# stnamjef/GenerativeDensification

Hardware: AMD Instinct MI355X
Metric: views/sec fwd+bwd @ 800x800 (higher is better)
Workload: dtype f32; 1 GPU; c4: BASELINE configs[3] per-GPU share: 2M densified-like Gaussians, 4 views/GPU 800x800, SH3, fwd+bwd; n_gaussians=2000000, layout=cube, order=random, views_per_gpu=4, sh_degree=3, parallelism=view-sharded x1, grad_allreduce=False, entry=render_views (all views of the shard, one node), activations fused into K1/K9, loss=folded into K6 epilogue / K7 prologue (clamp+MSE+0.1 mean depth+0.1 mean alpha)

## Files before the change

### generativedensification_amd/_debug.py

```python
import os as _os


def _int_env(name):
    return int(_os.environ[name]) if _os.environ.get(name) else None


RENDER_SIDE = int(_os.environ.get("GDR_RENDER_SIDE", "1"))
FWD_STREAMS = int(_os.environ.get("GDR_FWD_STREAMS", "4"))
BWD_STREAMS = _int_env("GDR_BWD_STREAMS")
BIN_STREAM = None
K7_VIEWS = _int_env("GDR_K7_VIEWS")
EARLY_CLEAR = True

SEG_LEN = _int_env("GDR_SEG_LEN")
DEEP_MAX_BUSY = None
DEEP_MIN_MEAN = _int_env("GDR_DEEP_MIN_MEAN")
FORCE_GLOBAL_SORT = False
SCATTER_MODE = int(_os.environ.get("GDR_SCATTER_MODE", "0"))
FORCE_RADIX_PARTITION = False
LAUNCH_HINTS = True

DEFER_D = _os.environ.get("GDR_DEFER_D", "1") != "0"
```

### generativedensification_amd/_lib.py

```python
from __future__ import annotations

import ctypes as C
import os

import torch

_HERE = os.path.dirname(os.path.abspath(__file__))
LIB_PATH = os.environ.get("GDR_LIB_PATH") or os.path.join(_HERE, "lib", "libgdr_hip.so")

GDR_OK = 0
GDR_IN_RAW_OPACITY, GDR_IN_RAW_SCALES, GDR_IN_RAW_ROTATIONS, GDR_IN_NO_DEPTH_TO_MEAN = 1, 2, 4, 8
GDR_MAX_VIEWS = 8
GDR_MAX_NODE_VIEWS = 256
ABI_VERSION = 17
GDR_SAME_AS_MAX, GDR_REUSE_MAX = 8, 32
GDR_DEFAULT_SEG_LEN = 256
GDR_ERR_WORKSPACE = -4


class GdrSettings(C.Structure):
    _fields_ = [("image_height", C.c_int32), ("image_width", C.c_int32), ("tanfovx", C.c_float),
                ("tanfovy", C.c_float), ("scale_modifier", C.c_float), ("sh_degree", C.c_int32),
                ("prefiltered", C.c_int32), ("debug", C.c_int32), ("bg", C.c_void_p),
                ("viewmatrix", C.c_void_p), ("projmatrix", C.c_void_p), ("campos", C.c_void_p)]
# ... 136 lines not shown
    _fields_ = [("N", C.c_int64), ("V", C.c_int32), ("C", C.c_int32), ("H", C.c_int32), ("W", C.c_int32),
                ("reserved", C.c_int32)]


GDR_SUBM_DTYPES = {"f16": 0, "bf16": 1, "f32": 2}
GDR_SUBM_MAX_TAPS, GDR_SUBM_MAX_CHANNELS, GDR_SUBM_MAX_POINTS = 125, 512, 1 << 30


GDR_SEG_ROWS, GDR_SEG_MAX_CHANNELS = 32, 65536
GDR_SEG_DTYPES = {"f16": 0, "bf16": 1, "f32": 2, "i64": 3}
GDR_SEG_OPS = {"sum": 0, "mean": 1, "min": 2, "max": 3}

GDR_NORM_DTYPES = {"f16": 0, "bf16": 1, "f32": 2}
GDR_NORM_ROWS, GDR_NORM_MAX_CHANNELS, GDR_NORM_MAX_SEGMENTS, GDR_NORM_MAX_FREQS, GDR_NORM_MAX_UPSCALE = 32, 1024, 1024, 16, 16


class GdrSubmArgs(C.Structure):
    _fields_ = [("N", C.c_int32), ("Cin", C.c_int32), ("Cout", C.c_int32), ("K", C.c_int32), ("dtype", C.c_int32),
                ("reserved", C.c_int32)]


_PROTOS = {
    "gdr_abi_version": (C.c_int, []),
    "gdr_last_error": (C.c_char_p, []),
    "gdr_geom_bytes": (C.c_size_t, [C.c_int32]),
    "gdr_binning_bytes": (C.c_size_t, [C.c_uint64]),
    "gdr_image_bytes": (C.c_size_t, [C.c_int32, C.c_int32]),
    "gdr_geom_carve": (C.c_int, [C.c_void_p, C.c_int32, C.POINTER(GdrGeom)]),
    "gdr_binning_carve": (C.c_int, [C.c_void_p, C.c_uint64, C.POINTER(GdrBinning)]),
    "gdr_binning_bytes_for": (C.c_size_t, [C.c_uint64, C.c_int32, C.c_int32, C.c_int32]),
    "gdr_binning_carve_for": (C.c_int, [C.c_void_p, C.c_uint64, C.c_int32, C.c_int32, C.c_int32, C.POINTER(GdrBinning)]),
    "gdr_build_tag": (C.c_char_p, []),
    "gdr_set_scatter_mode": (C.c_int32, [C.c_int32]),
    "gdr_words_differ": (C.c_int, [C.c_void_p, C.c_void_p, C.c_uint64, C.c_void_p, C.c_void_p]),
    "gdr_words_differ_multi": (C.c_int, [C.c_int32, C.POINTER(C.c_void_p), C.POINTER(C.c_void_p), C.POINTER(C.c_uint64), C.c_void_p,
                                         C.c_void_p]),
    "gdr_host_copy_begin": (C.c_int, [C.c_void_p, C.c_void_p, C.c_uint64, C.c_void_p, C.POINTER(C.c_void_p)]),
    "gdr_host_copy_wait": (C.c_int, [C.c_void_p]),
    "gdr_clear_async": (C.c_int, [C.c_void_p, C.c_uint64, C.c_void_p]),
    "gdr_image_carve": (C.c_int, [C.c_void_p, C.c_int32, C.c_int32, C.POINTER(GdrImage)]),
    "gdr_preprocess_forward": (C.c_int, [C.POINTER(GdrSettings), C.POINTER(GdrInputs), C.POINTER(GdrGeom),
                                         C.c_void_p, C.POINTER(C.c_uint32), C.c_void_p]),
    "gdr_render_forward": (C.c_int, [C.POINTER(GdrSettings), C.POINTER(GdrInputs), C.POINTER(GdrGeom),
                                     C.POINTER(GdrBinning), C.POINTER(GdrImage), C.c_uint64,
                                     C.POINTER(GdrOutputs), C.c_void_p]),
    "gdr_binning_forward": (C.c_int, [C.POINTER(GdrSettings), C.c_int32, C.POINTER(GdrGeom), C.POINTER(GdrBinning),
                                      C.POINTER(GdrImage), C.c_uint64, C.c_void_p, C.c_void_p]),
    "gdr_composite_forward": (C.c_int, [C.POINTER(GdrSettings), C.POINTER(GdrGeom), C.POINTER(GdrBinning),
                                        C.POINTER(GdrImage), C.POINTER(GdrOutputs), C.c_void_p]),
    "gdr_composite_forward_loss": (C.c_int, [C.POINTER(GdrSettings), C.POINTER(GdrGeom), C.POINTER(GdrBinning),
                                             C.POINTER(GdrImage), C.POINTER(GdrOutputs), C.c_void_p, C.c_float, C.c_float,
                                             C.c_void_p, C.c_void_p]),
    "gdr_composite_forward_views": (C.c_int, [C.c_int32, C.POINTER(GdrSettings), C.POINTER(GdrGeom), C.POINTER(GdrBinning),
                                              C.POINTER(GdrImage), C.POINTER(GdrOutputs), C.c_int32, C.POINTER(C.c_void_p),
                                              C.c_float, C.c_float, C.c_float, C.c_void_p, C.c_int32, C.c_void_p]),
    "gdr_render_backward_loss": (C.c_int, [C.POINTER(GdrSettings), C.c_int32, C.POINTER(GdrGeom), C.POINTER(GdrBinning),
                                           C.POINTER(GdrImage), C.c_void_p, C.c_void_p, C.c_float, C.c_float, C.c_void_p,
                                           C.c_void_p, C.c_void_p]),
    "gdr_forward": (C.c_int, [C.POINTER(GdrSettings), C.POINTER(GdrInputs), C.POINTER(GdrGeom),
                              C.POINTER(GdrBinning), C.POINTER(GdrImage), C.c_uint64,
                              C.POINTER(GdrOutputs), C.POINTER(C.c_uint32), C.c_void_p]),
    "gdr_view_plan_for": (C.c_int, [C.c_int32, C.c_int32, C.c_int32, C.c_int32, C.c_uint64, C.POINTER(GdrViewOpts),
                                    C.POINTER(GdrViewPlan)]),
    "gdr_forward_view": (C.c_int, [C.POINTER(GdrSettings), C.POINTER(GdrInputs), C.POINTER(GdrViewPlan), C.c_void_p,
                                   C.POINTER(GdrViewOpts), C.POINTER(GdrSameAs), C.POINTER(GdrOutputs),
                                   C.POINTER(GdrViewState), C.c_void_p]),
# ... 240 lines not shown
```

### generativedensification_amd/csrc/api.hip

```cpp
#include <stdio.h>
#include <string.h>

#include <atomic>
#include <cmath>
#include <mutex>
#include <unordered_map>
#include <vector>

#include "gdr_common.h"
#include "host_util.h"

namespace gdr {

static thread_local char g_err[512] = "";

void set_error(const char* what, hipError_t e) {
    snprintf(g_err, sizeof(g_err), "%s: %s (%d)", what, e == hipSuccess ? "" : hipGetErrorString(e), (int)e);
}

struct ProfRec { int id; hipEvent_t a, b; };
static bool g_prof_on = false;
static std::vector<ProfRec> g_prof_pending;
static std::vector<hipEvent_t> g_prof_pool;
static double g_prof_ms[GDR_K_COUNT];
// ... 264 lines not shown
        if (in->shs) {
            if (s->sh_degree < 0 || s->sh_degree > 3) { set_error("sh_degree must be 0..3", hipSuccess); return GDR_ERR_UNSUPPORTED; }
            if (in->M < (s->sh_degree + 1) * (s->sh_degree + 1)) { set_error("M < (sh_degree+1)^2", hipSuccess); return GDR_ERR_INVALID_ARG; }
            if (!s->campos) { set_error("campos NULL", hipSuccess); return GDR_ERR_INVALID_ARG; }
        }
    }
    return GDR_OK;
}

static int hip_fail(const char* what, hipError_t e) {
    set_error(what, e);
    return GDR_ERR_HIP;
}

static int debug_sync(const gdr_settings* s, const char* what, hipStream_t st) {
    if (!s->debug) return GDR_OK;
    hipError_t e = hipStreamSynchronize(st);
    if (e != hipSuccess) return hip_fail(what, e);
    return GDR_OK;
}

}

using namespace gdr;

extern "C" {

int gdr_abi_version(void) { return GDR_ABI_VERSION; }
#ifndef GDR_BUILD_TAG
#define GDR_BUILD_TAG "release"
#endif
const char* gdr_build_tag(void) { return GDR_BUILD_TAG; }
int32_t gdr_set_scatter_mode(int32_t mode) { return set_scatter_mode_default(mode); }
const char* gdr_last_error(void) { return g_err; }

size_t gdr_geom_bytes(int32_t N) { return carve_geom(nullptr, N, nullptr); }
size_t gdr_binning_bytes(uint64_t D) { return carve_binning(nullptr, D, nullptr); }
size_t gdr_image_bytes(int32_t H, int32_t W) { return carve_image(nullptr, H, W, nullptr); }

int gdr_geom_carve(void* base, int32_t N, gdr_geom* out) {
    if (!base || !out || ((uintptr_t)base & 255u)) { set_error("geom base NULL/unaligned", hipSuccess); return GDR_ERR_INVALID_ARG; }
    carve_geom(base, N, out);
    return GDR_OK;
}
int gdr_binning_carve(void* base, uint64_t D, gdr_binning* out) {
    if (!base || !out || ((uintptr_t)base & 255u)) { set_error("binning base NULL/unaligned", hipSuccess); return GDR_ERR_INVALID_ARG; }
    carve_binning(base, D, out);
    return GDR_OK;
}
size_t gdr_binning_bytes_for(uint64_t D, int32_t seg_len, int32_t N, int32_t tiles) {
    return carve_binning(nullptr, D, nullptr, seg_len, N, tiles);
}
int gdr_binning_carve_for(void* base, uint64_t D, int32_t seg_len, int32_t N, int32_t tiles, gdr_binning* out) {
    if (!base || !out || ((uintptr_t)base & 255u) || seg_len < 0 || N < 0 || tiles < 0) {
        set_error("binning base NULL/unaligned or negative seg_len / N / tiles", hipSuccess);
        return GDR_ERR_INVALID_ARG;
    }
    carve_binning(base, D, out, seg_len, N, tiles);
    return GDR_OK;
}
int gdr_image_carve(void* base, int32_t H, int32_t W, gdr_image* out) {
    if (!base || !out || ((uintptr_t)base & 255u)) { set_error("image base NULL/unaligned", hipSuccess); return GDR_ERR_INVALID_ARG; }
    carve_image(base, H, W, out);
    return GDR_OK;
}

// ... 1501 lines not shown
```

### generativedensification_amd/csrc/binning.hip

```cpp
#include <string.h>
#include <atomic>

#include "gdr_common.h"

namespace gdr {

namespace {

__device__ __forceinline__ uint32_t lane_id() { return threadIdx.x & 63u; }
__device__ __forceinline__ uint64_t lanemask_lt() { return (1ull << lane_id()) - 1ull; }

__device__ __forceinline__ uint32_t wave_incl_scan(uint32_t v) {
#pragma unroll
    for (int off = 1; off < 64; off <<= 1) {
        uint32_t t = __shfl_up(v, off, 64);
        if ((int)lane_id() >= off) v += t;
    }
    return v;
}

__device__ __forceinline__ uint32_t block_excl_scan(uint32_t v, uint32_t* lds, uint32_t* total) {
    const uint32_t incl = wave_incl_scan(v);
    const uint32_t w = threadIdx.x >> 6;
    if (lane_id() == 63) lds[w] = incl;
// ... 598 lines not shown
            uint32_t j = i + 1;
            while (j < L && kA[j] == kA[i]) ++j;
            if (j - i > GDR_TIE_SERIAL) {
                const uint32_t slot = atomicAdd(&runs[2 * GDR_TIE_RUNS], 1u);
                if (slot < GDR_TIE_RUNS) { runs[2 * slot] = i; runs[2 * slot + 1] = j - i; continue; }
            }
            for (uint32_t a = i + 1; a < j; ++a) {
                const uint32_t x = vA[a];
                uint32_t c = a;
                while (c > i && vA[c - 1] > x) { vA[c] = vA[c - 1]; --c; }
                vA[c] = x;
            }
        }
    }
    __syncthreads();
    const uint32_t nruns = min(runs[2 * GDR_TIE_RUNS], (uint32_t)GDR_TIE_RUNS);
    for (uint32_t r = 0; r < nruns; ++r) {
        const uint32_t i0 = runs[2 * r], Lr = runs[2 * r + 1];
        if constexpr (EPT > 0) {
            for (int shift = 0; shift < 32; shift += GDR_RADIX_BITS)
                tile_sort_pass_lds<NW, EPT>(vA + i0, vA + i0, Lr, 0u, shift, cnt, scan_lds);
            continue;
        }
        TileSortBufs t;
        t.kA = t.vA = vA + i0;
        t.kB = t.vB = vB + i0;
        for (int shift = 0; shift < 32; shift += GDR_RADIX_BITS) {
            tile_sort_pass<NW>(t, Lr, 0u, shift, cnt, scan_lds);
            uint32_t* x = t.kA; t.kA = t.vA = t.kB; t.kB = t.vB = x;
        }
    }
}

template <int CAP, int LMIN, int NW, bool TOP, bool PACKED>
__global__ __launch_bounds__(NW * GDR_WAVE) void tile_sort_kernel(const BinViews vs, int in, int ntiles) {
    const BinView& bv = vs.v[blockIdx.y];
    const uint2* __restrict__ ranges = bv.ranges;
    const uint64_t* __restrict__ keys_part = bv.keys[in];
    uint32_t* __restrict__ vals_part = bv.vals[in];
    uint32_t* __restrict__ vals_out = bv.vals[in ^ 1];
    uint32_t* __restrict__ scratch32 = bv.scratch32;
    const uint64_t D = bv.D;
    const uint32_t* __restrict__ tile_order = bv.tile_order;
    if (view_D(bv) == 0) return;
    constexpr uint32_t NT = NW * GDR_WAVE;
    __shared__ uint32_t lds_elems[2 * CAP];
    __shared__ uint32_t cnt[NW][GDR_RADIX];
    __shared__ uint32_t misc[8];
    __shared__ uint32_t mm[2 * NW];
    __shared__ uint32_t bstart[TOP ? GDR_RADIX + 1 : 1];
    __shared__ uint32_t bstart2[TOP ? GDR_RADIX + 1 : 1];
    __shared__ uint32_t tie_runs[2 * GDR_TIE_RUNS + 1];
    const uint32_t w = threadIdx.x >> 6, lane = lane_id();

    auto min_max = [&](uint32_t& kmin, uint32_t& kmax) __attribute__((always_inline)) {
#pragma unroll
        for (int off = 32; off > 0; off >>= 1) {
            kmin = min(kmin, (uint32_t)__shfl_xor((int)kmin, off, 64));
            kmax = max(kmax, (uint32_t)__shfl_xor((int)kmax, off, 64));
        }
        if (lane == 0) { mm[w] = kmin; mm[NW + w] = kmax; }
        __syncthreads();
        for (int k = 0; k < NW; ++k) { kmin = min(kmin, mm[k]); kmax = max(kmax, mm[NW + k]); }
    };
    auto sort_in_lds = [&](auto key_at, auto val_at, uint32_t o, uint32_t Lc) __attribute__((always_inline)) {
        __syncthreads();
        constexpr int EPT = CAP / (int)NT;
        uint32_t* const kA = lds_elems;
        uint32_t* const vA = lds_elems + CAP;
        uint32_t kmin = 0xFFFFFFFFu, kmax = 0u;
        for (uint32_t i = threadIdx.x; i < Lc; i += NT) {
            const uint32_t k = key_at(i);
            kA[i] = k;
            vA[i] = val_at(i);
            kmin = min(kmin, k);
            kmax = max(kmax, k);
        }
        min_max(kmin, kmax);
        const uint32_t span = kmax - kmin;
        const int nbits = span ? 32 - __builtin_clz(span) : 0;
        for (int shift = 0; shift < nbits; shift += GDR_RADIX_BITS)
            tile_sort_pass_lds<NW, EPT>(kA, vA, Lc, kmin, shift, cnt, misc);
        tile_sort_ties<NW, EPT>(kA, vA, nullptr, Lc, cnt, misc, tie_runs);
        for (uint32_t i = threadIdx.x; i < Lc; i += NT) vals_out[o + i] = vA[i];
    };

    for (uint32_t slot = blockIdx.x; slot < (uint32_t)ntiles; slot += gridDim.x) {
        const uint32_t tile = LMIN > 0 ? tile_order[slot] : slot;
        const uint2 rg = ranges[tile];
        const uint32_t L = rg.y - rg.x;
        if (LMIN > 0 && (L >> 4) < ((uint32_t)LMIN >> 4)) return;
        if (L <= (uint32_t)LMIN || (!TOP && L > (uint32_t)CAP)) continue;
        if (L <= (uint32_t)CAP) {
            const uint64_t* kp = keys_part + rg.x;
            const uint32_t* vp = vals_part + rg.x;
            if constexpr (PACKED)
                sort_in_lds([kp](uint32_t i) { return (uint32_t)kp[i]; }, [kp](uint32_t i) { return (uint32_t)(kp[i] >> 32); }, rg.x, L);
            else
                sort_in_lds([kp](uint32_t i) { return (uint32_t)kp[i]; }, [vp](uint32_t i) { return vp[i]; }, rg.x, L);
            continue;
        }
        if constexpr (TOP) {
            uint32_t* const kA = scratch32 + rg.x;
            uint32_t* const kB = scratch32 + D + rg.x;
            uint32_t* const vA = vals_part + rg.x;
            uint32_t* const vB = vals_out + rg.x;
            __syncthreads();
            uint32_t kmin = 0xFFFFFFFFu, kmax = 0u;
            for (uint32_t i = threadIdx.x; i < L; i += NT) {
                const uint32_t k = (uint32_t)keys_part[rg.x + i];
                if constexpr (!PACKED) kA[i] = k;
// ... 58 lines not shown
                        sort_in_lds([kc](uint32_t i) { return kc[i]; }, [vc](uint32_t i) { return vc[i]; }, rg.x + s0 + s1, Lcc);
                        continue;
                    }
                    TileSortBufs h;
                    h.kA = kA + s0 + s1; h.vA = vA + s0 + s1; h.kB = kB + s0 + s1; h.vB = vB + s0 + s1;
                    finish_global(h, Lcc, sh2, rg.x + s0 + s1);
                }
            }
        }
    }
}

}

size_t sort_hist_bytes(uint64_t D) {
    const uint64_t nblk = (D + GDR_SORT_TILE - 1) / GDR_SORT_TILE;
    return (size_t)((nblk > 0 ? nblk : 1) * GDR_RADIX + GDR_RADIX) * sizeof(uint32_t);
}

hipError_t launch_scan_block_sums(const gdr_geom* g, int N, hipStream_t st) {
    const int nb = div_up(N, GDR_BLOCK);
    GDR_LAUNCH(GDR_K_SCAN, scan_block_sums_kernel, dim3(1), dim3(GDR_BLOCK), st, g->block_sums, nb,
                       g->num_rendered);
    return hipGetLastError();
}

static std::atomic<int32_t> g_scatter_mode{GDR_SCATTER_AUTO};
int32_t scatter_mode_default() { return g_scatter_mode.load(std::memory_order_relaxed); }
int32_t set_scatter_mode_default(int32_t mode) {
    if (mode < 0 || mode > (GDR_SCATTER_MODE_MASK | GDR_SCATTER_LINEAR_ROWS) || (mode & GDR_SCATTER_MODE_MASK) == 3) mode = GDR_SCATTER_AUTO;
    return g_scatter_mode.exchange(mode, std::memory_order_relaxed);
}

void fill_bin_views(BinViews* vs, int V, const gdr_geom* geoms, const gdr_binning* bins, const gdr_image* imgs,
                    const uint64_t* D, const int32_t* const* radii) {
    memset(vs, 0, sizeof(*vs));
    for (int v = 0; v < V; ++v) {
        BinView& b = vs->v[v];
        const gdr_geom& g = geoms[v];
        const gdr_binning& bn = bins[v];
        b.radii = radii ? radii[v] : nullptr;
        b.depths = g.depths; b.rect = (const int4*)g.rect; b.tiles_touched = g.tiles_touched;
        b.block_offs = bn.global_sort ? g.block_sums : g.block_offs;
        b.keys[0] = bn.keys[0]; b.keys[1] = bn.keys[1]; b.vals[0] = bn.values[0]; b.vals[1] = bn.values[1];
        b.hist = bn.hist; b.scratch32 = bn.scratch32; b.tile_hist = bn.tile_hist; b.hist_width = bn.hist_width;
        b.from_totals = 0;
        b.scatter_mode = bn.scatter_mode != 0 ? bn.scatter_mode : scatter_mode_default();
        b.ranges = (uint2*)imgs[v].ranges; b.tile_order = imgs[v].tile_order; b.seg_base = imgs[v].seg_base;
        b.seg_extra = (uint2*)bn.seg_extra; b.seg_count = bn.seg_count;
        b.D = D[v]; b.nblk = (uint32_t)((D[v] + GDR_SORT_TILE - 1) / GDR_SORT_TILE);
        b.d_dev = bn.d_dev;
        b.stats_out = bn.stats_out; b.hint_long = bn.hint_long; b.hint_medium = bn.hint_medium;
        b.seg_len = bn.seg_len; b.seg_cap = bn.seg_cap;
        b.deep_max_busy = (uint32_t)(bn.deep_max_busy > 0 ? bn.deep_max_busy : 0);
        b.deep_min_mean = (uint32_t)(bn.deep_min_mean > 0 ? bn.deep_min_mean : GDR_DEEP_MIN_MEAN);
    }
}

static uint64_t max_D(const BinViews& vs, int V) {
    uint64_t m = 0;
    for (int v = 0; v < V; ++v) m = vs.v[v].D > m ? vs.v[v].D : m;
    return m;
}

hipError_t launch_duplicate_views(const BinViews& vs, int V, int N, int W, int H, hipStream_t st) {
    const int tiles = tile_grid_x(W) * tile_grid_y(H);
// ... 81 lines not shown
    if (mode == GDR_SCATTER_AUTO && stage_cap > 0u) {
        uint64_t est = 0;
        for (int v = 0; v < V; ++v) {
            const uint64_t d = vs.v[v].d_dev ? vs.v[v].D * 2 / 3 : vs.v[v].D;
            est = d > est ? d : est;
        }
        if (est / (uint64_t)nwg > (uint64_t)stage_cap * 9 / 10) stage_cap = 0u;
    }
    if (stage_cap > 0u) {
        const size_t lds = (size_t)stage_cap * sizeof(uint64_t) + 2 * (size_t)tiles * sizeof(uint32_t);
        hipError_t e = hipFuncSetAttribute((const void*)tile_scatter_staged_kernel, hipFuncAttributeMaxDynamicSharedMemorySize, (int)lds);
        if (e != hipSuccess) return e;
        prof_begin(GDR_K_TILE_SCATTER, st);
        hipLaunchKernelGGL(tile_scatter_staged_kernel, dim3(bin_grid(nwg, per_xcd), V), dim3(GDR_BIN_THREADS), lds, st, vs, N, gx,
                           tiles, chunk, tstride, nwg, per_xcd, stage_cap);
        prof_end(GDR_K_TILE_SCATTER, st);
        return hipGetLastError();
    }
    prof_begin(GDR_K_TILE_SCATTER, st);
    hipLaunchKernelGGL(tile_scatter_kernel, dim3(bin_grid(nwg, per_xcd), V), dim3(GDR_BIN_THREADS), (size_t)tiles * sizeof(uint32_t),
                       st, vs, N, gx, tiles, chunk, tstride, nwg, per_xcd);
    prof_end(GDR_K_TILE_SCATTER, st);
    return hipGetLastError();
}

#ifndef GDR_TSORT_MEDIUM_WAVES
#define GDR_TSORT_MEDIUM_WAVES 8
#endif
#ifndef GDR_TSORT_NO_LONG
#define GDR_TSORT_NO_LONG 0
#endif
hipError_t launch_tile_sort_views(const BinViews& vs, int V, int in, int tiles, bool packed, hipStream_t st) {
    if (max_D(vs, V) == 0) return hipSuccess;
    int g_long = tiles < 256 ? tiles : 256, g_medium = tiles < 512 ? tiles : 512;
    const int h_long = merged_hint(vs, V, true), h_medium = merged_hint(vs, V, false);
    if (h_long > 0 && h_long < g_long) g_long = h_long;
    if (h_medium > 0 && h_medium < g_medium) g_medium = h_medium;
    bool no_long = true;
    for (int v = 0; v < V; ++v) no_long = no_long && vs.v[v].hint_long < 0;
    if (GDR_TSORT_NO_LONG) no_long = true;
    constexpr int MW = GDR_TSORT_MEDIUM_WAVES;
    if (packed) {
        if (!no_long)
            GDR_LAUNCH(GDR_K_TILE_SORT_LONG, (tile_sort_kernel<GDR_TSORT_LARGE, GDR_TSORT_MEDIUM, 16, true, true>),
                       dim3(g_long, V), dim3(16 * GDR_WAVE), st, vs, in, tiles);
        if (no_long)
            GDR_LAUNCH(GDR_K_TILE_SORT_LONG, (tile_sort_kernel<GDR_TSORT_MEDIUM, GDR_TSORT_SMALL, MW, true, true>),
                       dim3(g_medium, V), dim3(MW * GDR_WAVE), st, vs, in, tiles);
        else
            GDR_LAUNCH(GDR_K_TILE_SORT_LONG, (tile_sort_kernel<GDR_TSORT_MEDIUM, GDR_TSORT_SMALL, MW, false, true>),
                       dim3(g_medium, V), dim3(MW * GDR_WAVE), st, vs, in, tiles);
        GDR_LAUNCH(GDR_K_TILE_SORT, (tile_sort_kernel<GDR_TSORT_SMALL, 0, 4, false, true>), dim3(tiles, V), dim3(GDR_BLOCK), st,
                   vs, in, tiles);
        return hipGetLastError();
    }
    GDR_LAUNCH(GDR_K_TILE_SORT_LONG, (tile_sort_kernel<GDR_TSORT_LARGE, GDR_TSORT_MEDIUM, 16, true, false>),
               dim3(g_long, V), dim3(16 * GDR_WAVE), st, vs, in, tiles);
    GDR_LAUNCH(GDR_K_TILE_SORT_LONG, (tile_sort_kernel<GDR_TSORT_MEDIUM, GDR_TSORT_SMALL, 8, false, false>),
               dim3(g_medium, V), dim3(8 * GDR_WAVE), st, vs, in, tiles);
    GDR_LAUNCH(GDR_K_TILE_SORT, (tile_sort_kernel<GDR_TSORT_SMALL, 0, 4, false, false>), dim3(tiles, V), dim3(GDR_BLOCK), st, vs,
               in, tiles);
    return hipGetLastError();
}

}
```

### generativedensification_amd/csrc/gdr_common.h

```cpp
#pragma once
#include <hip/hip_runtime.h>
#include <stdint.h>

#include "../../include/gdr.h"
#include "../../include/gsr.h"

#define GDR_WAVE 64
#define GDR_BLOCK 256
#define GDR_TILE_PIX (GDR_TILE * GDR_TILE)

#define GDR_SORT_ITEMS 16
#define GDR_SORT_TILE (GDR_BLOCK * GDR_SORT_ITEMS)
#define GDR_RADIX_BITS 8
#define GDR_RADIX (1 << GDR_RADIX_BITS)

enum {
    GDR_K_PREPROCESS_FWD = 0,
    GDR_K_SCAN,
    GDR_K_DUPLICATE,
    GDR_K_SORT_HIST,
    GDR_K_SORT_ROWSCAN,
    GDR_K_SORT_SCATTER,
    GDR_K_RANGES,
    GDR_K_RENDER_FWD,
// ... 45 lines not shown
hipError_t launch_preprocess_fwd_views(int V, const gdr_settings* s, const gdr_inputs* in,
                                       const gdr_geom* geoms, int32_t* const* radii, hipStream_t st);
hipError_t launch_preprocess_bwd_views(int V, const gdr_settings* s, const gdr_inputs* in,
                                       const gdr_geom* geoms, const int32_t* const* radii,
                                       float* const* grad_recs, const gdr_grad_outputs* go,
                                       hipStream_t st);
hipError_t launch_mark_visible(int N, const float* means3D, const float* view, uint8_t* present,
                               hipStream_t st);
hipError_t launch_scan_block_sums(const gdr_geom* g, int N, hipStream_t st);
struct BinView {
    const int32_t* radii; const float* depths; const int4* rect; const uint32_t* tiles_touched; const uint32_t* block_offs;
    uint64_t* keys[2]; uint32_t* vals[2]; uint32_t* hist; uint32_t* scratch32;
    uint2* ranges; uint32_t* tile_order; uint32_t* seg_base; uint2* seg_extra; uint32_t* seg_count;
    uint64_t D; uint32_t nblk; int32_t seg_len, seg_cap; uint32_t deep_max_busy, deep_min_mean;
    const uint32_t* d_dev;
    uint32_t* stats_out;
    int32_t hint_long, hint_medium;
    uint32_t* tile_hist; int32_t hist_width;
    int32_t from_totals;
    int32_t scatter_mode;
};
#define GDR_BIN_MAX_TILES 16384
#define GDR_BIN_MAX_WIDTH 256
#define GDR_TSORT_SMALL 2048
#define GDR_TSORT_MEDIUM 4096
#define GDR_TSORT_LARGE 16384
#define GDR_SCATTER_AUTO 0
#define GDR_SCATTER_DIRECT 1
#define GDR_SCATTER_STAGED 2
#define GDR_SCATTER_MODE_MASK 3
#define GDR_SCATTER_LINEAR_ROWS 4
int32_t scatter_mode_default();
int32_t set_scatter_mode_default(int32_t mode);
struct BinViews { BinView v[GDR_MAX_VIEWS]; };
void fill_bin_views(BinViews* vs, int V, const gdr_geom* geoms, const gdr_binning* bins, const gdr_image* imgs,
                    const uint64_t* D, const int32_t* const* radii);
hipError_t launch_duplicate_views(const BinViews& vs, int V, int N, int W, int H, hipStream_t st);
hipError_t launch_sort_views(const BinViews& vs, int V, int lo, int hi, int* sorted, hipStream_t st);
hipError_t launch_ranges_views(const BinViews& vs, int V, int cur, int tiles, hipStream_t st);
hipError_t launch_tile_sort_views(const BinViews& vs, int V, int in, int tiles, bool packed, hipStream_t st);
hipError_t launch_tile_count_scan(const BinViews& vs, int V, int N, int W, int H, hipStream_t st);
hipError_t launch_tile_scatter(const BinViews& vs, int V, int N, int W, int H, hipStream_t st);
hipError_t launch_tile_order_views(const BinViews& vs, int V, int tiles, hipStream_t st);
#define GDR_SEG_STATE_FLOATS (10 * GDR_BLOCK)
#define GDR_DEEP_MIN_MEAN 2560
hipError_t launch_render_fwd(const gdr_settings* s, const gdr_geom* g, const gdr_binning* bin,
                             const gdr_image* img, const gdr_outputs* out, hipStream_t st);
hipError_t launch_render_fwd_loss(const gdr_settings* s, const gdr_geom* g, const gdr_binning* bin,
                                  const gdr_image* img, const gdr_outputs* out, const float* target, float w_depth,
                                  float w_alpha, float* loss, hipStream_t st);
hipError_t launch_render_fwd_lossgrad(const gdr_settings* s, const gdr_geom* g, const gdr_binning* bin,
                                      const gdr_image* img, const float* target, float go_scale, float* loss,
                                      float* dL_dcolor, hipStream_t st);
hipError_t launch_render_fwd_views(int V, const gdr_settings* s, const gdr_geom* g, const gdr_binning* bin, const gdr_image* img,
                                   const gdr_outputs* outs, int loss_mode, const float* const* targets, float w_depth,
                                   float w_alpha, float go_scale, float* losses, int interleave, hipStream_t st);
hipError_t launch_topk_absgrad(int N, const float* grad, const uint8_t* cand, int k, void* workspace,
                               uint8_t* mask, int32_t* idx, hipStream_t st);
size_t select_workspace_bytes();
void surfel_render_bwd_set_pairs(int pairs);
void render_bwd_set_pairs(int pairs);
hipError_t launch_render_bwd_loss(const gdr_settings* s, const gdr_geom* g, const gdr_binning* bin,
                                  const gdr_image* img, const float* color, const float* target, float w_depth,
                                  float w_alpha, const float* go, float* grad_rec, hipStream_t st);
hipError_t launch_render_bwd_mean2d_loss(const gdr_settings* s, const gdr_geom* g, const gdr_binning* bin,
                                         const gdr_image* img, const float* color, const float* target, const float* go,
// ... 76 lines not shown
```

### generativedensification_amd/rasterizer.py

```python
from __future__ import annotations

import ctypes as C
import math
import os as _os
import threading
from typing import NamedTuple

import torch
from torch import nn

from . import _debug as K
from . import _lib as L
from . import _marshal as M
from . import viewgroup


class GaussianRasterizationSettings(NamedTuple):
    image_height: int
    image_width: int
    tanfovx: float
    tanfovy: float
    bg: torch.Tensor
    scale_modifier: float
    viewmatrix: torch.Tensor
# ... 162 lines not shown
    def groups(self):
        return [(lo, min(L.GDR_MAX_VIEWS, self.n - lo)) for lo in range(0, self.n, L.GDR_MAX_VIEWS)]

    def _side_of(self, k):
        return self.side[k % len(self.side)]

    def stream(self, k):
        if self.side:
            return C.c_void_p(self._side_of(k).cuda_stream)
        return C.c_void_p(self.main.cuda_stream)

    def k9_stream(self, lo, n):
        if self.side:
            for sd in {self._side_of(k) for k in range(lo, lo + n)}:
                done = torch.cuda.Event()
                done.record(sd)
                self.main.wait_event(done)
        return C.c_void_p(self.main.cuda_stream)

    def join(self):
        if self.side:
            for sd in self.side:
                done = torch.cuda.Event()
                done.record(sd)
                self.main.wait_event(done)


class GroupMismatch(RuntimeError):
    """A later call of a render group was handed values that differ from the group's (viewgroup.py falls back to an
    independent node for that call)."""


_SCATTER_MODE_SENT = [0]


def _push_scatter_mode():
    m = int(K.SCATTER_MODE)
    if m != _SCATTER_MODE_SENT[0]:
        L.load().gdr_set_scatter_mode(m)
        _SCATTER_MODE_SENT[0] = m


def _view_opts():
    _push_scatter_mode()
    return L.GdrViewOpts(-1 if K.SEG_LEN is None else max(0, int(K.SEG_LEN)) // 256 * 256,
                         -1 if K.DEEP_MAX_BUSY is None else max(0, int(K.DEEP_MAX_BUSY)),
                         -1 if K.DEEP_MIN_MEAN is None else max(0, int(K.DEEP_MIN_MEAN)),
                         int(K.FORCE_GLOBAL_SORT), int(K.FORCE_RADIX_PARTITION), int(not K.LAUNCH_HINTS))


def view_opts_tuple():
    _push_scatter_mode()
    return (-1 if K.SEG_LEN is None else max(0, int(K.SEG_LEN)) // 256 * 256,
            -1 if K.DEEP_MAX_BUSY is None else max(0, int(K.DEEP_MAX_BUSY)),
            -1 if K.DEEP_MIN_MEAN is None else max(0, int(K.DEEP_MIN_MEAN)),
            int(K.FORCE_GLOBAL_SORT), int(K.FORCE_RADIX_PARTITION), int(not K.LAUNCH_HINTS))


def forward_view_native(call, s, inp, N, H, W, surfel, out, same_as, dev, stream):
    lib = L.load()
    opts, plan, vs = _view_opts(), L.GdrViewPlan(), L.GdrViewState()
    same = None
    if same_as:
        same = L.GdrSameAs()
        same.n = len(same_as)
        for k, (t, ref) in enumerate(same_as):
            same.a[k], same.b[k], same.n_bytes[k] = t.data_ptr(), ref.data_ptr(), t.numel() * 4
        same = C.byref(same)
    exact = 0
    for _ in range(4):
        L.check(lib.gdr_view_plan_for(N, H, W, int(surfel), exact, C.byref(opts), C.byref(plan)), "gdr_view_plan_for")
        if not K.DEFER_D and not exact:
            plan.have_binning = 0
# ... 343 lines not shown
    with _HIST_LOCK:
        t = _LAUNCH_STATS.get(key)
        if t is None:
            if len(_LAUNCH_STATS) >= 1024:
                return None, None
            try:
                t = torch.full((V, 4), -1, dtype=torch.int32).pin_memory()
            except RuntimeError:
                return None, None
            _LAUNCH_STATS[key] = t
        seen = [r for r in t.tolist() if r[0] >= 0]
        if not seen:
            return t, None
        n_long, n_medium, deep = max(r[0] for r in seen), max(r[1] for r in seen), any(r[2] for r in seen)
        st = _HINT_STATE.setdefault(key, [0, 0, 0])
        st[0], st[1] = max(n_long, st[0] * 9 // 10), max(n_medium, st[1] * 9 // 10)
        st[2] = 8 if deep else max(0, st[2] - 1)
        st = list(st)
    return t, (-1 if st[0] == 0 else max(16, st[0] + st[0] // 4 + 1), max(32, st[1] + st[1] // 4 + 1), int(st[2] == 0),
               max(r[3] for r in seen))


def _carve_binning(lib, st, entries, tiles, d_dev=None, stats=None, hints=None):
    seg_len = _seg_len_for(entries if d_dev is None else int(entries / D_SLACK), tiles, None if hints is None else hints[3])
    need = lib.gdr_binning_bytes_for(entries, seg_len, st.N, tiles)
    if st.bin_buf is None or st.bin_buf.numel() < need:
        st.bin_buf = torch.empty(need, dtype=torch.uint8, device=st.geom_buf.device)
    L.check(lib.gdr_binning_carve_for(st.bin_buf.data_ptr(), entries, seg_len, st.N, tiles, C.byref(st.bin)),
            "gdr_binning_carve_for")
    if K.FORCE_RADIX_PARTITION:
        st.bin.tile_hist, st.bin.hist_width = None, 0
    st.bin.global_sort = int(K.FORCE_GLOBAL_SORT)
    st.bin.scatter_mode = int(K.SCATTER_MODE)
    st.bin.d_dev = d_dev
    st.D = entries
    if K.DEEP_MAX_BUSY is not None:
        st.bin.deep_max_busy = max(0, int(K.DEEP_MAX_BUSY))
    if K.DEEP_MIN_MEAN is not None:
        st.bin.deep_min_mean = max(0, int(K.DEEP_MIN_MEAN))
    if hints is not None:
        st.bin.hint_long, st.bin.hint_medium, st.bin.hint_no_deep = hints[:3]
    if stats is not None:
        st.bin.stats_out = stats.data_ptr()


def _forward_views_impl(means3D, means2D, sh, opacities, scales, rotations, settings_list, flags, loss_spec=None):
    lib = L.load()
    _require_hip(means3D, "means3D")
    dev = means3D.device
    in_dtypes = tuple(t.dtype for t in (means3D, means2D, sh, opacities, scales, rotations))
    means3D, sh = _f32(means3D, dev), _f32(sh, dev)
    opacities, scales, rotations = _f32(opacities, dev), _f32(scales, dev), _f32(rotations, dev)
    N, M, V = int(means3D.shape[0]), int(sh.shape[1]), len(settings_list)
    H, W = int(settings_list[0].image_height), int(settings_list[0].image_width)
    if any(int(rs.image_height) != H or int(rs.image_width) != W for rs in settings_list):
        raise RuntimeError("render_views: all views must share one image size")
    if V > L.GDR_MAX_NODE_VIEWS:
        raise RuntimeError(f"render_views: {V} views in one node; one native forward call takes at most {L.GDR_MAX_NODE_VIEWS} "
                           "(include/gdr.h GDR_MAX_NODE_VIEWS) — split the view list")
    e = empty_f32(dev)
    keep = [means3D, opacities, sh, e, scales, rotations, e]
    f32 = dict(dtype=torch.float32, device=dev)
    lossgrad = loss_spec is not None and loss_spec[0] == "lossgrad"
    colors = [torch.empty(3, H, W, **f32) for _ in range(V)]
    depths = [None if lossgrad else torch.empty(1, H, W, **f32) for _ in range(V)]
    alphas = [None if lossgrad else torch.empty(1, H, W, **f32) for _ in range(V)]
# ... 391 lines not shown
```

### include/gdr.h

```cpp
#ifndef GDR_H
#define GDR_H

#include <stddef.h>
#include <stdint.h>

#ifdef __cplusplus
extern "C" {
#endif

#define GDR_ABI_VERSION 17

#define GDR_OK 0
#define GDR_ERR_INVALID_ARG (-1)
#define GDR_ERR_HIP (-2)
#define GDR_ERR_UNSUPPORTED (-3)
#define GDR_ERR_WORKSPACE (-4)

#define GDR_MAX_GAUSSIANS (1 << 27)
#define GDR_MAX_RENDERED 0xFFFFFFFFull

#define GDR_DEFAULT_DEEP_MAX_BUSY 768
#define GDR_DEFAULT_SEG_LEN 256
#define GDR_TILE 16

// ... 79 lines not shown
} gdr_image;

typedef struct gdr_outputs {
    float* color;
    float* depth;
    float* alpha;
    int32_t* radii;
} gdr_outputs;

typedef struct gdr_grad_inputs {
    const float* dL_dcolor;
    const float* dL_ddepth;
    const float* dL_dalpha;
} gdr_grad_inputs;

typedef struct gdr_grad_outputs {
    float* dL_dmeans3D;
    float* dL_dmeans2D;
    float* dL_dshs;
    float* dL_dcolors;
    float* dL_dopacities;
    float* dL_dscales;
    float* dL_drotations;
    float* dL_dcov3D;
    float* scratch;
    int32_t accumulate;
    int32_t reserved;
} gdr_grad_outputs;

int gdr_abi_version(void);
const char* gdr_last_error(void);
const char* gdr_build_tag(void);
int32_t gdr_set_scatter_mode(int32_t mode);

size_t gdr_geom_bytes(int32_t N);
size_t gdr_binning_bytes(uint64_t D);
size_t gdr_image_bytes(int32_t H, int32_t W);
int gdr_geom_carve(void* base, int32_t N, gdr_geom* out);
int gdr_binning_carve(void* base, uint64_t D, gdr_binning* out);
size_t gdr_binning_bytes_for(uint64_t D, int32_t seg_len, int32_t N, int32_t tiles);
int gdr_binning_carve_for(void* base, uint64_t D, int32_t seg_len, int32_t N, int32_t tiles, gdr_binning* out);
int gdr_image_carve(void* base, int32_t H, int32_t W, gdr_image* out);

int gdr_preprocess_forward(const gdr_settings* s, const gdr_inputs* in, const gdr_geom* geom,
                           int32_t* radii, uint32_t* num_rendered_host, void* stream);

int gdr_render_forward(const gdr_settings* s, const gdr_inputs* in, const gdr_geom* geom,
                       gdr_binning* bin, const gdr_image* img, uint64_t D,
                       const gdr_outputs* out, void* stream);

int gdr_binning_forward(const gdr_settings* s, int32_t N, const gdr_geom* geom, gdr_binning* bin, const gdr_image* img,
                        uint64_t D, const int32_t* radii, void* stream);
int gdr_composite_forward(const gdr_settings* s, const gdr_geom* geom, const gdr_binning* bin, const gdr_image* img,
                          const gdr_outputs* out, void* stream);

int gdr_composite_forward_loss(const gdr_settings* s, const gdr_geom* geom, const gdr_binning* bin, const gdr_image* img,
                               const gdr_outputs* out, const float* target, float w_depth, float w_alpha, float* loss,
                               void* stream);
int gdr_render_backward_loss(const gdr_settings* s, int32_t N, const gdr_geom* geom, const gdr_binning* bin,
                             const gdr_image* img, const float* color, const float* target, float w_depth, float w_alpha,
                             const float* g, float* grad_rec, void* stream);

int gdr_composite_forward_views(int32_t V, const gdr_settings* s, const gdr_geom* geoms, const gdr_binning* bins,
                                const gdr_image* imgs, const gdr_outputs* outs, int32_t loss_mode,
                                const float* const* targets, float w_depth, float w_alpha, float go_scale, float* losses,
                                int32_t interleave, void* stream);
// ... 308 lines not shown
```

Before: 1516 views/s.

## Add bucket-count sort path for small and medium per-tile key sorts

For tiles at or below the medium capacity, the tile sort now builds a 4096-bucket histogram over the key range using packed 16-bit LDS counters and scatters entries into buckets. It then ranks each element within its bucket by direct comparison, replacing the multi-pass LDS radix sort when no bucket exceeds 16 entries. Tiles whose buckets overflow fall back to the radix path and increment a device-side fallback counter. The change also adds occupancy hints to launch bounds, and grows the LDS counter array, which could lower occupancy or add work on dense tiles.

Measured after the change: 1550 views/s, median of 6. 1.02x the previous value.

```diff
diff --git a/generativedensification_amd/_debug.py b/generativedensification_amd/_debug.py
--- a/generativedensification_amd/_debug.py
+++ b/generativedensification_amd/_debug.py
@@ -17,7 +17,16 @@
 DEEP_MIN_MEAN = _int_env("GDR_DEEP_MIN_MEAN")
 FORCE_GLOBAL_SORT = False
 SCATTER_MODE = int(_os.environ.get("GDR_SCATTER_MODE", "0"))
+TILE_SORT_MODE = int(_os.environ.get("GDR_TILE_SORT_MODE", "0"))
 FORCE_RADIX_PARTITION = False
 LAUNCH_HINTS = True
 
 DEFER_D = _os.environ.get("GDR_DEFER_D", "1") != "0"
+
+
+def tile_sort_fallbacks(reset=True):
+    from . import _lib
+    n = int(_lib.load().gdr_debug_tile_sort_fallbacks(1 if reset else 0))
+    if n < 0:
+        raise RuntimeError("gdr_debug_tile_sort_fallbacks failed")
+    return n
diff --git a/generativedensification_amd/_lib.py b/generativedensification_amd/_lib.py
--- a/generativedensification_amd/_lib.py
+++ b/generativedensification_amd/_lib.py
@@ -192,6 +192,8 @@
     "gdr_binning_carve_for": (C.c_int, [C.c_void_p, C.c_uint64, C.c_int32, C.c_int32, C.c_int32, C.POINTER(GdrBinning)]),
     "gdr_build_tag": (C.c_char_p, []),
     "gdr_set_scatter_mode": (C.c_int32, [C.c_int32]),
+    "gdr_set_tile_sort_mode": (C.c_int32, [C.c_int32]),
+    "gdr_debug_tile_sort_fallbacks": (C.c_int64, [C.c_int32]),
     "gdr_words_differ": (C.c_int, [C.c_void_p, C.c_void_p, C.c_uint64, C.c_void_p, C.c_void_p]),
     "gdr_words_differ_multi": (C.c_int, [C.c_int32, C.POINTER(C.c_void_p), C.POINTER(C.c_void_p), C.POINTER(C.c_uint64), C.c_void_p,
                                          C.c_void_p]),
diff --git a/generativedensification_amd/csrc/api.hip b/generativedensification_amd/csrc/api.hip
--- a/generativedensification_amd/csrc/api.hip
+++ b/generativedensification_amd/csrc/api.hip
@@ -320,6 +320,8 @@
 #endif
 const char* gdr_build_tag(void) { return GDR_BUILD_TAG; }
 int32_t gdr_set_scatter_mode(int32_t mode) { return set_scatter_mode_default(mode); }
+int32_t gdr_set_tile_sort_mode(int32_t mode) { return set_tile_sort_mode_default(mode); }
+int64_t gdr_debug_tile_sort_fallbacks(int32_t reset) { return tile_sort_fallbacks(reset); }
 const char* gdr_last_error(void) { return g_err; }
 
 size_t gdr_geom_bytes(int32_t N) { return carve_geom(nullptr, N, nullptr); }
diff --git a/generativedensification_amd/csrc/binning.hip b/generativedensification_amd/csrc/binning.hip
--- a/generativedensification_amd/csrc/binning.hip
+++ b/generativedensification_amd/csrc/binning.hip
@@ -654,8 +654,13 @@
     }
 }
 
+#define GDR_TSORT_BUCKETS 4096
+#define GDR_TSORT_BUCKET_MAX 16
+#define GDR_TSORT_FB_SLOTS 32
+__device__ uint32_t g_tsort_fallbacks[GDR_TSORT_FB_SLOTS * 16];
+
 template <int CAP, int LMIN, int NW, bool TOP, bool PACKED>
-__global__ __launch_bounds__(NW * GDR_WAVE) void tile_sort_kernel(const BinViews vs, int in, int ntiles) {
+__global__ __launch_bounds__(NW * GDR_WAVE, NW == 4 ? 5 : 4) void tile_sort_kernel(const BinViews vs, int in, int ntiles, int bucket) {
     const BinView& bv = vs.v[blockIdx.y];
     const uint2* __restrict__ ranges = bv.ranges;
     const uint64_t* __restrict__ keys_part = bv.keys[in];
@@ -667,7 +672,12 @@
     if (view_D(bv) == 0) return;
     constexpr uint32_t NT = NW * GDR_WAVE;
     __shared__ uint32_t lds_elems[2 * CAP];
-    __shared__ uint32_t cnt[NW][GDR_RADIX];
+    constexpr bool BUCKET = CAP <= GDR_TSORT_MEDIUM;
+    constexpr int BWORDS = GDR_TSORT_BUCKETS / 2;
+    constexpr int CNT_WORDS = (BUCKET && NW * GDR_RADIX < BWORDS) ? BWORDS : NW * GDR_RADIX;
+    __shared__ uint32_t cnt_words[CNT_WORDS];
+    uint32_t (*const cnt)[GDR_RADIX] = reinterpret_cast<uint32_t (*)[GDR_RADIX]>(cnt_words);
+    __shared__ uint32_t bsc[2 * NW];
     __shared__ uint32_t misc[8];
     __shared__ uint32_t mm[2 * NW];
     __shared__ uint32_t bstart[TOP ? GDR_RADIX + 1 : 1];
@@ -691,14 +701,119 @@
         uint32_t* const kA = lds_elems;
         uint32_t* const vA = lds_elems + CAP;
         uint32_t kmin = 0xFFFFFFFFu, kmax = 0u;
-        for (uint32_t i = threadIdx.x; i < Lc; i += NT) {
-            const uint32_t k = key_at(i);
-            kA[i] = k;
-            vA[i] = val_at(i);
-            kmin = min(kmin, k);
-            kmax = max(kmax, k);
-        }
-        min_max(kmin, kmax);
+        bool in_lds = false;
+        if constexpr (BUCKET) {
+            if (bucket) {
+                constexpr int WPT = BWORDS / (int)NT;
+                uint32_t key[EPT], val[EPT];
+#pragma unroll
+                for (int j = 0; j < EPT; ++j) {
+                    const uint32_t i = threadIdx.x + (uint32_t)j * NT;
+                    const bool valid = i < Lc;
+                    key[j] = valid ? key_at(i) : 0u;
+                    val[j] = valid ? val_at(i) : 0u;
+                    if (valid) { kmin = min(kmin, key[j]); kmax = max(kmax, key[j]); }
+                }
+#pragma unroll
+                for (int k = 0; k < WPT; ++k) cnt_words[threadIdx.x + (uint32_t)k * NT] = 0u;
+                min_max(kmin, kmax);
+                const uint32_t span = kmax - kmin;
+                const int nbits = span ? 32 - __builtin_clz(span) : 0;
+                const int bshift = nbits > 12 ? nbits - 12 : 0;
+#pragma unroll
+                for (int j = 0; j < EPT; ++j) {
+                    const uint32_t b = (key[j] - kmin) >> bshift;
+                    if (threadIdx.x + (uint32_t)j * NT < Lc) atomicAdd(&cnt_words[b >> 1], 1u << ((b & 1u) * 16u));
+                }
+                __syncthreads();
+                uint32_t cw[WPT], sum = 0u, big = 0u;
+#pragma unroll
+                for (int k = 0; k < WPT; ++k) {
+                    cw[k] = cnt_words[threadIdx.x * WPT + k];
+                    const uint32_t c0 = cw[k] & 0xFFFFu, c1 = cw[k] >> 16;
+                    sum += c0 + c1;
+                    big = max(big, max(c0, c1));
+                }
+                const uint32_t incl = wave_incl_scan(sum);
+#pragma unroll
+                for (int off = 32; off > 0; off >>= 1) big = max(big, (uint32_t)__shfl_xor((int)big, off, 64));
+                if (lane == 63) bsc[w] = incl;
+                if (lane == 0) bsc[NW + w] = big;
+                __syncthreads();
+                uint32_t base = incl - sum;
+                for (uint32_t k = 0; k < (uint32_t)NW; ++k) {
+                    if (k < w) base += bsc[k];
+                    big = max(big, bsc[NW + k]);
+                }
+                if (big <= (uint32_t)GDR_TSORT_BUCKET_MAX) {
+                    uint32_t s = base;
+#pragma unroll
+                    for (int k = 0; k < WPT; ++k) {
+                        const uint32_t c0 = cw[k] & 0xFFFFu, c1 = cw[k] >> 16;
+                        cnt_words[threadIdx.x * WPT + k] = s | ((s + c0) << 16);
+                        s += c0 + c1;
+                    }
+                    __syncthreads();
+#pragma unroll
+                    for (int j = 0; j < EPT; ++j) {
+                        const uint32_t b = (key[j] - kmin) >> bshift, sh = (b & 1u) * 16u;
+                        if (threadIdx.x + (uint32_t)j * NT < Lc) {
+                            const uint32_t slot = (atomicAdd(&cnt_words[b >> 1], 1u << sh) >> sh) & 0xFFFFu;
+                            kA[slot] = key[j];
+                            vA[slot] = val[j];
+                        }
+                    }
+                    __syncthreads();
+                    const uint16_t* const ends = reinterpret_cast<const uint16_t*>(cnt_words);
+                    uint32_t pos[EPT], lim[EPT], rank[EPT];
+#pragma unroll
+                    for (int j = 0; j < EPT; ++j) {
+                        const uint32_t i = threadIdx.x + (uint32_t)j * NT;
+                        const bool valid = i < Lc;
+                        key[j] = valid ? kA[i] : kmin;
+                        val[j] = valid ? vA[i] : 0u;
+                        const uint32_t b = (key[j] - kmin) >> bshift;
+                        const uint32_t e = valid ? ends[b] : 0u;
+                        pos[j] = (valid && b > 0u) ? ends[b - 1u] : 0u;
+                        lim[j] = e - pos[j] >= 2u && valid ? e : pos[j];
+                        rank[j] = 0u;
+                    }
+                    for (uint32_t t = 0; t < (uint32_t)GDR_TSORT_BUCKET_MAX; ++t) {
+                        bool more = false;
+#pragma unroll
+                        for (int j = 0; j < EPT; ++j) {
+                            const bool in = pos[j] + t < lim[j];
+                            const uint32_t q = in ? pos[j] + t : 0u;
+                            const uint32_t kq = kA[q], vq = vA[q];
+                            rank[j] += (in && (kq < key[j] || (kq == key[j] && vq < val[j]))) ? 1u : 0u;
+                            more = more || in;
+                        }
+                        if (!__any(more)) break;
+                    }
+#pragma unroll
+                    for (int j = 0; j < EPT; ++j)
+                        if (threadIdx.x + (uint32_t)j * NT < Lc) vals_out[o + pos[j] + rank[j]] = val[j];
+                    return;
+                }
+                if (threadIdx.x == 0) atomicAdd(&g_tsort_fallbacks[(blockIdx.x % GDR_TSORT_FB_SLOTS) * 16], 1u);
+#pragma unroll
+                for (int j = 0; j < EPT; ++j) {
+                    const uint32_t i = threadIdx.x + (uint32_t)j * NT;
+                    if (i < Lc) { kA[i] = key[j]; vA[i] = val[j]; }
+                }
+                in_lds = true;
+            }
+        }
+        if (!in_lds) {
+            for (uint32_t i = threadIdx.x; i < Lc; i += NT) {
+                const uint32_t k = key_at(i);
+                kA[i] = k;
+                vA[i] = val_at(i);
+                kmin = min(kmin, k);
+                kmax = max(kmax, k);
+            }
+            min_max(kmin, kmax);
+        }
         const uint32_t span = kmax - kmin;
         const int nbits = span ? 32 - __builtin_clz(span) : 0;
         for (int shift = 0; shift < nbits; shift += GDR_RADIX_BITS)
@@ -823,6 +938,25 @@
     return g_scatter_mode.exchange(mode, std::memory_order_relaxed);
 }
 
+static std::atomic<int32_t> g_tile_sort_mode{GDR_TSORT_AUTO};
+int32_t tile_sort_mode_default() { return g_tile_sort_mode.load(std::memory_order_relaxed); }
+int32_t set_tile_sort_mode_default(int32_t mode) {
+    if (mode < 0 || mode > GDR_TSORT_BUCKET) mode = GDR_TSORT_AUTO;
+    return g_tile_sort_mode.exchange(mode, std::memory_order_relaxed);
+}
+int64_t tile_sort_fallbacks(int32_t reset) {
+    uint32_t h[GDR_TSORT_FB_SLOTS * 16];
+    if (hipDeviceSynchronize() != hipSuccess) return -1;
+    if (hipMemcpyFromSymbol(h, HIP_SYMBOL(g_tsort_fallbacks), sizeof(h)) != hipSuccess) return -1;
+    int64_t n = 0;
+    for (int k = 0; k < GDR_TSORT_FB_SLOTS; ++k) n += h[k * 16];
+    if (reset) {
+        memset(h, 0, sizeof(h));
+        if (hipMemcpyToSymbol(HIP_SYMBOL(g_tsort_fallbacks), h, sizeof(h)) != hipSuccess) return -1;
+    }
+    return n;
+}
+
 void fill_bin_views(BinViews* vs, int V, const gdr_geom* geoms, const gdr_binning* bins, const gdr_image* imgs,
                     const uint64_t* D, const int32_t* const* radii) {
     memset(vs, 0, sizeof(*vs));
@@ -970,6 +1104,7 @@
 #endif
 hipError_t launch_tile_sort_views(const BinViews& vs, int V, int in, int tiles, bool packed, hipStream_t st) {
     if (max_D(vs, V) == 0) return hipSuccess;
+    const int bucket = tile_sort_mode_default() != GDR_TSORT_RADIX ? 1 : 0;
     int g_long = tiles < 256 ? tiles : 256, g_medium = tiles < 512 ? tiles : 512;
     const int h_long = merged_hint(vs, V, true), h_medium = merged_hint(vs, V, false);
     if (h_long > 0 && h_long < g_long) g_long = h_long;
@@ -981,23 +1116,23 @@
     if (packed) {
         if (!no_long)
             GDR_LAUNCH(GDR_K_TILE_SORT_LONG, (tile_sort_kernel<GDR_TSORT_LARGE, GDR_TSORT_MEDIUM, 16, true, true>),
-                       dim3(g_long, V), dim3(16 * GDR_WAVE), st, vs, in, tiles);
+                       dim3(g_long, V), dim3(16 * GDR_WAVE), st, vs, in, tiles, bucket);
         if (no_long)
             GDR_LAUNCH(GDR_K_TILE_SORT_LONG, (tile_sort_kernel<GDR_TSORT_MEDIUM, GDR_TSORT_SMALL, MW, true, true>),
-                       dim3(g_medium, V), dim3(MW * GDR_WAVE), st, vs, in, tiles);
+                       dim3(g_medium, V), dim3(MW * GDR_WAVE), st, vs, in, tiles, bucket);
         else
             GDR_LAUNCH(GDR_K_TILE_SORT_LONG, (tile_sort_kernel<GDR_TSORT_MEDIUM, GDR_TSORT_SMALL, MW, false, true>),
-                       dim3(g_medium, V), dim3(MW * GDR_WAVE), st, vs, in, tiles);
+                       dim3(g_medium, V), dim3(MW * GDR_WAVE), st, vs, in, tiles, bucket);
         GDR_LAUNCH(GDR_K_TILE_SORT, (tile_sort_kernel<GDR_TSORT_SMALL, 0, 4, false, true>), dim3(tiles, V), dim3(GDR_BLOCK), st,
-                   vs, in, tiles);
+                   vs, in, tiles, bucket);
         return hipGetLastError();
     }
     GDR_LAUNCH(GDR_K_TILE_SORT_LONG, (tile_sort_kernel<GDR_TSORT_LARGE, GDR_TSORT_MEDIUM, 16, true, false>),
-               dim3(g_long, V), dim3(16 * GDR_WAVE), st, vs, in, tiles);
+               dim3(g_long, V), dim3(16 * GDR_WAVE), st, vs, in, tiles, bucket);
     GDR_LAUNCH(GDR_K_TILE_SORT_LONG, (tile_sort_kernel<GDR_TSORT_MEDIUM, GDR_TSORT_SMALL, 8, false, false>),
-               dim3(g_medium, V), dim3(8 * GDR_WAVE), st, vs, in, tiles);
+               dim3(g_medium, V), dim3(8 * GDR_WAVE), st, vs, in, tiles, bucket);
     GDR_LAUNCH(GDR_K_TILE_SORT, (tile_sort_kernel<GDR_TSORT_SMALL, 0, 4, false, false>), dim3(tiles, V), dim3(GDR_BLOCK), st, vs,
-               in, tiles);
+               in, tiles, bucket);
     return hipGetLastError();
 }
 
diff --git a/generativedensification_amd/csrc/gdr_common.h b/generativedensification_amd/csrc/gdr_common.h
--- a/generativedensification_amd/csrc/gdr_common.h
+++ b/generativedensification_amd/csrc/gdr_common.h
@@ -101,6 +101,12 @@
 #define GDR_SCATTER_LINEAR_ROWS 4
 int32_t scatter_mode_default();
 int32_t set_scatter_mode_default(int32_t mode);
+#define GDR_TSORT_AUTO 0
+#define GDR_TSORT_RADIX 1
+#define GDR_TSORT_BUCKET 2
+int32_t tile_sort_mode_default();
+int32_t set_tile_sort_mode_default(int32_t mode);
+int64_t tile_sort_fallbacks(int32_t reset);
 struct BinViews { BinView v[GDR_MAX_VIEWS]; };
 void fill_bin_views(BinViews* vs, int V, const gdr_geom* geoms, const gdr_binning* bins, const gdr_image* imgs,
                     const uint64_t* D, const int32_t* const* radii);
diff --git a/generativedensification_amd/rasterizer.py b/generativedensification_amd/rasterizer.py
--- a/generativedensification_amd/rasterizer.py
+++ b/generativedensification_amd/rasterizer.py
@@ -218,6 +218,7 @@
 
 
 _SCATTER_MODE_SENT = [0]
+_TILE_SORT_MODE_SENT = [0]
 
 
 def _push_scatter_mode():
@@ -225,6 +226,10 @@
     if m != _SCATTER_MODE_SENT[0]:
         L.load().gdr_set_scatter_mode(m)
         _SCATTER_MODE_SENT[0] = m
+    m = int(K.TILE_SORT_MODE)
+    if m != _TILE_SORT_MODE_SENT[0]:
+        L.load().gdr_set_tile_sort_mode(m)
+        _TILE_SORT_MODE_SENT[0] = m
 
 
 def _view_opts():
@@ -634,6 +639,7 @@
         st.bin.tile_hist, st.bin.hist_width = None, 0
     st.bin.global_sort = int(K.FORCE_GLOBAL_SORT)
     st.bin.scatter_mode = int(K.SCATTER_MODE)
+    _push_scatter_mode()
     st.bin.d_dev = d_dev
     st.D = entries
     if K.DEEP_MAX_BUSY is not None:
diff --git a/include/gdr.h b/include/gdr.h
--- a/include/gdr.h
+++ b/include/gdr.h
@@ -135,6 +135,8 @@
 const char* gdr_last_error(void);
 const char* gdr_build_tag(void);
 int32_t gdr_set_scatter_mode(int32_t mode);
+int32_t gdr_set_tile_sort_mode(int32_t mode);
+int64_t gdr_debug_tile_sort_fallbacks(int32_t reset);
 
 size_t gdr_geom_bytes(int32_t N);
 size_t gdr_binning_bytes(uint64_t D);
```
